# xiaochuanle/NECAT

Measured on AMD Instinct MI355X. Metric: overlaps/sec (all-vs-all, index build + seeding + banded Myers extension -> M4), higher is better.
Workload: dtype u64

## Files before the change

### necat_amd/csrc/knobs.h

```cpp
#pragma once
#include <stddef.h>
#include <stdint.h>
#include <stdlib.h>
#include <string>

#define NECAT_KNOBS(NUM, INT, SET, STR) \
     \
    NUM(index_lds,         int,    "NECAT_INDEX_LDS",         1, 0, ~0ull)            \
    NUM(split_threads,     ull,    "NECAT_SPLIT_THREADS",     512, 0, ~0ull)          \
    INT(index_own_offsets,         "NECAT_INDEX_OWN_OFFSETS", 0)                      \
    INT(index_emit_big,            "NECAT_INDEX_EMIT_BIG",    -1)                     \
    INT(index_dense_bases,         "NECAT_INDEX_DENSE_BASES", 0)                      \
    INT(no_lend,                   "NECAT_NO_LEND",          0)                      \
     \
    NUM(seed_budget,       ull,    "NECAT_SEED_BUDGET",       48ull << 20, 0, ~0ull)  \
    NUM(seed_wave,         int,    "NECAT_SEED_WAVE",         1, 0, ~0ull)            \
    NUM(seed_kst,          int,    "NECAT_SEED_KST",          1, 0, ~0ull)            \
    INT(seed_debug,                "NECAT_SEED_DEBUG",        0)                      \
    INT(chain_wave,                "NECAT_CHAIN_WAVE",        1)                      \
    SET(seed_clear_kernel,         "NECAT_SEED_CLEAR_KERNEL")                         \
     \
    NUM(batch_cap,         u32,    "NECAT_BATCH",             786432, 64, ~0ull)      \
     \
    NUM(ext_overlap,       u32,    "NECAT_EXT_OVERLAP",       1, 0, ~0ull) \
    NUM(ext_overlap_min,   u32,    "NECAT_EXT_OVERLAP_MIN",   0, 0, ~0ull) \
    NUM(ext_overlap_pct,   u32,    "NECAT_EXT_OVERLAP_PCT",   100, 0, 100) \
    NUM(ext_overlap_split, u32,    "NECAT_EXT_OVERLAP_SPLIT", 20, 5, 95) \
    NUM(ext_overlap_order, u32,    "NECAT_EXT_ORDER",         1, 0, ~0ull)            \
    NUM(ext_lanes,         u32,    "NECAT_EXT_LANES",         2, 1, kMaxExtLanes)     \
    INT(lane1_prio,                "NECAT_LANE1_PRIO",        1)                      \
    INT(serial,                    "NECAT_SERIAL",            0)                      \
    INT(stream_prio,               "NECAT_STREAM_PRIO",       0)                      \
     \
    NUM(coop_threshold,    u32,    "NECAT_COOP_THRESHOLD",    0xffffffffu, 0, ~0ull)  \
    NUM(coop_filter,       int,    "NECAT_COOP_FILTER",       1, 0, ~0ull)            \
    NUM(single_pass,       u32,    "NECAT_SINGLE_PASS",       4096, 0, ~0ull)         \
    NUM(sort_b,            int,    "NECAT_SORT_B",            1, 0, ~0ull)            \
    NUM(fast,              int,    "NECAT_FAST",              1, 0, ~0ull)            \
    NUM(fast16,            int,    "NECAT_FAST16",            0, 0, ~0ull)            \
    NUM(band_pool,         size_t, "NECAT_BAND_POOL_MB",      16384, 0, ~0ull)        \
    NUM(walk,              int,    "NECAT_WALK",              0, 0, ~0ull)            \
    NUM(walk_wave,         u32,    "NECAT_WALK_WAVE",         12288, 0, ~0ull)        \
    NUM(tail_fused,        u32,    "NECAT_TAIL_FUSED",        512, 0, ~0ull)          \
    NUM(dbg,               int,    "NECAT_DBG",               0, 0, ~0ull)            \
     \
    NUM(rcwalk,            u32,    "NECAT_RCWALK",            512, 0, ~0ull)          \
    NUM(rc_pool,           size_t, "NECAT_RC_POOL_MB",        8192, 1, ~0ull)         \
    NUM(rc_carry,          u32,    "NECAT_RC_CARRY",          1, 0, ~0ull)            \
    NUM(rc_listb,          u32,    "NECAT_RC_LISTB",          1, 0, ~0ull)            \
    NUM(rc_ragged,         u32,    "NECAT_RC_RAGGED",         1, 0, ~0ull)            \
    NUM(rc_merge,          u32,    "NECAT_RC_MERGE",          1, 0, ~0ull)            \
    NUM(frag_fuse,         u32,    "NECAT_FRAG_FUSE",         1, 0, ~0ull)            \
    NUM(item_sort,         u32,    "NECAT_ITEM_SORT",         1, 0, ~0ull)            \
    SET(rc_ckg_all,                "NECAT_RC_CKG_ALL")                                \
    NUM(rc_maxdist,        int,    "NECAT_RC_MAXDIST",        1 << 20, 0, ~0ull)      \
    NUM(ck_lds,            u32,    "NECAT_CK_LDS",            0, 0, ~0ull)            \
    NUM(ck_post,           u32,    "NECAT_CK_POST",           1, 0, ~0ull)            \
    NUM(ckr_fast,          u32,    "NECAT_CKR_FAST",          1, 0, ~0ull)            \
    NUM(rc_fastb,          u32,    "NECAT_RC_FASTB",          1, 0, ~0ull)            \
    NUM(rc_prio,           u32,    "NECAT_RC_PRIO",           1, 0, ~0ull)            \
     \
    NUM(rc_pipe,           u32,    "NECAT_RC_PIPE",           1, 1, 8) \
    NUM(rc_pipe_min,       u32,    "NECAT_RC_PIPE_MIN",       49152, 0, ~0ull) \
    NUM(rc_dbg,            u32,    "NECAT_RC_DBG",            0, 0, ~0ull)            \
    NUM(rc_prefetch,       u32,    "NECAT_RC_PREFETCH",       0, 0, ~0ull)            \
    NUM(rc_ww,             u32,    "NECAT_RC_WW",             1, 0, ~0ull)            \
    NUM(rc3_band,          ull,    "NECAT_RC3_BAND",          32, 0, ~0ull)           \
    NUM(rc3_min,           u32,    "NECAT_RC3_MIN",           160000, 0, ~0ull)       \
     \
    NUM(batch_chunk,       u32,    "NECAT_BATCH_CHUNK",       65536, 0, ~0ull)        \
    SET(batch_rc,                  "NECAT_BATCH_RC")                                  \
     \
    NUM(asm_rc,            u32,    "NECAT_ASM_RC",            1, 0, ~0ull)            \
    NUM(asm_rc_pool,       size_t, "NECAT_ASM_RC_POOL_MB",    2048, 256, ~0ull)       \
    NUM(asm_lane,          int,    "NECAT_ASM_LANE",          0, 0, ~0ull)            \
    NUM(asm_vote_budget,   ull,    "NECAT_ASM_VOTE_BUDGET",   16ull << 20, 1024, ~0ull)   \
    NUM(asm_seed_budget,   ull,    "NECAT_ASM_SEED_BUDGET",   32ull << 20, 1024, ~0ull)   \
    NUM(asm_ends_device,   int,    "NECAT_ASM_ENDS_DEVICE",   0, 0, 1)                \
    NUM(asm_ends_diags,    u32,    "NECAT_ASM_ENDS_DIAGS",    128, 4, 2048)           \
    SET(asm_no_overlap,            "NECAT_ASM_NO_OVERLAP")                            \
    STR(asm_dump_votes,            "NECAT_ASM_DUMP_VOTES")                            \
     \
    INT(cns_spec_extra,            "NECAT_CNS_SPEC_EXTRA",    1)                      \
    NUM(cns_spec_cover,    int,    "NECAT_CNS_SPEC",          12, 0, ~0ull)           \
    NUM(cns_device,        int,    "NECAT_CNS_DEVICE",        1, 0, 1)                \
    STR(cns_reads,                 "NECAT_CNS_READS")                                 \
    NUM(cns_chunk_bases,   ull,    "NECAT_CNS_CHUNK_BASES",   1ull << 31, 1, 1ull << 40)    \
    NUM(cns_tag_budget,    ull,    "NECAT_CNS_TAG_BUDGET",   32ull << 20, 1, 1ull << 30)   \
    NUM(cns_tol_scale,     ull,    "NECAT_CNS_TOL_SCALE",     1, 1, 1ull << 40)       \
    NUM(nw_device,         int,    "NECAT_NW_DEVICE",         0, 0, 1)                \
    NUM(nw_pool,           size_t, "NECAT_NW_POOL_MB",        1024, 1, 1ull << 20)    \
    NUM(dalign_device,     int,    "NECAT_DALIGN_DEVICE",     0, 0, 1)                \
    NUM(dalign_diags,      u32,    "NECAT_DALIGN_DIAGS",      512, 4, 2048)           \
    NUM(rm_rescue_device,  int,    "NECAT_RM_RESCUE_DEVICE",  0, 0, 1)                \
    NUM(ctg_seed_lds,      u32,    "NECAT_CTG_SEED_LDS",      512, 0, 2048)           \
    NUM(ctg_seed_budget,   ull,    "NECAT_CTG_SEED_BUDGET",   4ull << 20, 1, 1ull << 28)   \
    NUM(ctg_seed_job_max,  ull,    "NECAT_CTG_SEED_JOB_MAX",  16384, 1, 1ull << 28)        \
    INT(cns_threads,               "NECAT_CNS_THREADS",       32)                     \
    STR(comm,                      "NECAT_COMM")                                      \
    NUM(trace,             int,    "NECAT_TRACE",             0, 0, ~0ull)

namespace necat {

struct KnobSet { bool set; int v; };

struct Knobs {
    typedef uint32_t u32;
    typedef unsigned long long ull;
#define NECAT_KNOB_NUM(field, type, name, dflt, lo, hi) type field;
#define NECAT_KNOB_INT(field, name, dflt) int field;
#define NECAT_KNOB_SET(field, name) KnobSet field;
#define NECAT_KNOB_STR(field, name) std::string field;
    NECAT_KNOBS(NECAT_KNOB_NUM, NECAT_KNOB_INT, NECAT_KNOB_SET, NECAT_KNOB_STR)
};

extern thread_local const Knobs* tl_knobs;
inline const Knobs& knob() { return *tl_knobs; }

inline void index_plan_env(double* link_gbs, int* shard)
{
    const char *g = getenv("NECAT_XGMI_GBS"), *s = getenv("NECAT_INDEX_SHARD");
    *link_gbs = g && atof(g) > 0 ? atof(g) : 100.0; *shard = s ? atoi(s) != 0 : -1;
}

}
```

### necat_amd/csrc/necat_hip.hip

```cpp
#include <algorithm>
#include <chrono>
#include <memory>
#include <mutex>
#include <unordered_map>
#include <time.h>
#include <unistd.h>
#include <numeric>
#include <atomic>
#include <type_traits>

#ifdef NECAT_BUILD_CROSSCHECK
#define NECAT_XCHECK 1
#else
#define NECAT_XCHECK 0
#endif

#include "runtime.h"
#include "index_kernels.h"
#include "volume_kernels.h"
#include "seed_kernels.h"
#include "pcan_kernels.h"
#include "trim_kernels.h"
#include "ext_kernels.h"
#include "ext_tail.h"
#include "ext_rcwalk.h"
#include "ext_rcwalk3.h"
#include "asm_kernels.h"
#include "asm_coop.h"
#include "asm_plan.h"
#include "host_bases.h"
#include "host_threads.h"
#include "cns_loop.h"
#include "cns_rescue.h"
#include "cns_consensus.h"
#include "cns_dev_kernels.h"
#include "ctg_consensus.h"
#include "ctg_dev_kernels.h"
#include "ctg_seed.h"
#include "ctg_seed_kernels.h"
#include "ctg_extend.h"
#include "nw_kernels.h"
#include "dal_kernels.h"
#include "asm_ends_core.h"
#include "rm_host.h"
#include "rescue_pair.h"
#include "comm.h"
#include "pair_sched.h"


namespace necat { thread_local const Knobs* tl_knobs = nullptr; }
using namespace necat;

#define NECAT_RETIRED(ctx, what) return necat::set_err(ctx, NECAT_ERR_ARG, "%s: a cross-check path this library is built without (it is in libnecat_hip_xcheck.so, -DNECAT_BUILD_CROSSCHECK)", what)

static_assert(SC_COUNT <= (int)(sizeof(necat_ctx::scratch) / sizeof(necat::DevBuf)), "a ScratchId without an arena");

namespace {

int ensure_zeroed(necat_ctx* ctx, DevBuf& b, size_t bytes, hipStream_t s)
{
    const void* before = b.p; const size_t cap0 = b.cap;
    int rc = buf_ensure(ctx, b, bytes);
    if (rc) return rc;
    if (b.p != before || b.cap != cap0) { hipError_t e = hipMemsetAsync(b.p, 0, b.cap, s); if (e != hipSuccess) return set_err(ctx, NECAT_ERR_DEVICE, "memset failed"); }
    return NECAT_OK;
}

inline unsigned grid_for(uint64_t n, unsigned block, unsigned cap = 1u << 20)
{
    uint64_t g = (n + block - 1) / block;
    if (g < 1) g = 1;
    if (g > cap) g = cap;
    return (unsigned)g;
}

DevVolume dev_view(const necat_volume* v)
{
    DevVolume d; d.bases = v->bases; d.seq_off = v->seq_off; d.nbases = v->nbases; d.nseq = v->nseq;
    return d;
}


void finish_knobs(necat::Knobs& K)
{
    if (!K.rc_carry) { K.rc_listb = K.rc_ragged = 0; K.rc_maxdist = std::min(K.rc_maxdist, kRcMaxDist); }
    K.rc3_band = K.rc3_band == 16 ? 16 : 32;
    K.split_threads = K.split_threads == 256 ? 256 : 512;
    K.rc_dbg &= 6u;
    K.band_pool <<= 20; K.rc_pool <<= 20; K.asm_rc_pool <<= 20; K.nw_pool <<= 20;
    if (K.cns_threads <= 0) K.cns_threads = 32;
}

void read_knobs(necat::Knobs& K)
{
#define READ_NUM(field, type, name, dflt, lo, hi) { const char* e = getenv(name); K.field = (decltype(K.field))std::min<Knobs::ull>(hi, std::max<Knobs::ull>(lo, e ? strtoull(e, nullptr, 10) : (Knobs::ull)(dflt))); }
#define READ_INT(field, name, dflt) { const char* e = getenv(name); K.field = e ? atoi(e) : (dflt); }
#define READ_SET(field, name) { const char* e = getenv(name); K.field.set = e != nullptr; K.field.v = e ? atoi(e) : 0; }
#define READ_STR(field, name) { const char* e = getenv(name); K.field = e ? e : ""; }
    NECAT_KNOBS(READ_NUM, READ_INT, READ_SET, READ_STR)
    finish_knobs(K);
}

template <class T> int knob_text(char* buf, size_t n, T v) { if (std::is_signed<T>::value) snprintf(buf, n, "%lld", (long long)v); else snprintf(buf, n, "%llu", (unsigned long long)v); return NECAT_OK; }
int knob_text(char* buf, size_t n, const necat::KnobSet& v) { if (v.set) snprintf(buf, n, "%d", v.v); else buf[0] = 0; return NECAT_OK; }
int knob_text(char* buf, size_t n, const std::string& v) { snprintf(buf, n, "%s", v.c_str()); return NECAT_OK; }

double wall_ms() { struct timespec ts; clock_gettime(CLOCK_MONOTONIC, &ts); return ts.tv_sec * 1e3 + ts.tv_nsec * 1e-6; }

int fetch_words(necat_ctx* ctx, const necat_volume* v, std::vector<u64>* words)
{
    words->resize((v->nbases + 31) / 32 + 1);
    NECAT_HIP(ctx, hipMemcpy(words->data(), v->bases, (words->size() - 1) * 8, hipMemcpyDeviceToHost));
    return NECAT_OK;
}

int fetch_read_words(necat_ctx* ctx, const necat_volume* v, uint64_t id, std::vector<u64>* words, u64* word0)
{
    const u64 b = v->h_seq_off[id], e = v->h_seq_off[id + 1];
    *word0 = b >> 5;
    words->resize(e == b ? 0 : ((e - 1) >> 5) - *word0 + 1);
    if (!words->empty()) NECAT_HIP(ctx, hipMemcpy(words->data(), v->bases + *word0, words->size() * 8, hipMemcpyDeviceToHost));
    return NECAT_OK;
}

necat_host::BaseWords host_view(const necat_volume* v, const std::vector<u64>& words, u64 word0 = 0)
{
    necat_host::BaseWords b; b.w = words.data(); b.word0 = word0; b.seq_off = v->h_seq_off.data();
    return b;
}

unsigned call_threads(const necat_ctx* ctx, int host_threads)
{
    const unsigned want = host_threads ? (unsigned)std::min(host_threads, 256) : (unsigned)ctx->knobs.cns_threads;
    return std::max(1u, std::min(want, std::min(necat_host::hardware_threads(), 256u)));
}

struct SeqAt { int64_t k; u64 begin, len; };
bool seq_at(const necat_volume* v, int64_t id, int64_t start_id, SeqAt* s)
{
    s->k = id - start_id;
    if (s->k < 0 || (uint64_t)s->k >= v->nseq) return false;
    s->begin = v->h_seq_off[s->k]; s->len = v->h_seq_off[s->k + 1] - s->begin;
    return true;
}

int ctg_segment_check(necat_ctx* ctx, const necat_volume* contigs, const necat_ctg_segment& S, uint64_t s, int min_size, const char* what)
{
    if (S.size < 0 || S.from < 0 || S.ovlp_begin > S.ovlp_end) return set_err(ctx, NECAT_ERR_ARG, "segment %lu: bad size, start or %s range", (unsigned long)s, what);
    if ((int64_t)S.size >= necat_host::ctg::kMaxSegment) return set_err(ctx, NECAT_ERR_ARG, "segment %lu has %d bases: 2^24 or more", (unsigned long)s, S.size);
    if (S.size < min_size) return set_err(ctx, NECAT_ERR_ARG, "segment %lu has %d bases: fewer than %d, the reference has no defined answer", (unsigned long)s, S.size, min_size);
    SeqAt c;
    if (contigs && (!seq_at(contigs, S.ctg_id, 0, &c) || (u64)S.from + (u64)S.size > c.len)) return set_err(ctx, NECAT_ERR_ARG, "segment %lu leaves its contig", (unsigned long)s);
    return NECAT_OK;
}
static_assert(necat_host::ctg::kMaxSegment == necat_host::ctg_seed::kMaxSegment, "one bound on a segment for both contig stages");

}

#include "stage_ck_round.inl"

extern "C" {

void necat_default_options(necat_map_options* o)
{
    o->kmer_size = 15; o->scan_window = 10; o->kmer_cnt_cutoff = 500; o->block_size = 2000;
    o->block_score_cutoff = 3; o->num_candidates = 500; o->align_size_cutoff = 500;
    o->ddfs_cutoff = 0.25; o->error = 0.5; o->num_output = 500; o->num_threads = 1;
    o->job = 1; o->binary_output = 0; o->use_hdr_as_id = 1;
}

static thread_local char g_create_err[256] = "no context";
#define NECAT_CREATE_FAIL(code, ...) do { snprintf(g_create_err, sizeof g_create_err, __VA_ARGS__); return (code); } while (0)

int necat_ctx_create(int device_id, necat_ctx** out)
{
    if (!out) return NECAT_ERR_ARG;
    *out = nullptr;
    int ndev = 0;
    if (hipGetDeviceCount(&ndev) != hipSuccess || ndev <= 0) { (void)hipGetLastError(); NECAT_CREATE_FAIL(NECAT_ERR_DEVICE, "no usable HIP device (there is no CPU fallback)"); }
    if (device_id < 0 || device_id >= ndev) NECAT_CREATE_FAIL(NECAT_ERR_ARG, "device %d of %d", device_id, ndev);
    if (hipSetDevice(device_id) != hipSuccess) NECAT_CREATE_FAIL(NECAT_ERR_DEVICE, "hipSetDevice(%d) failed", device_id);
    necat_ctx* ctx = new necat_ctx();
    ctx->device = device_id;
    read_knobs(ctx->knobs);
#if !NECAT_XCHECK
    if (ctx->knobs.rc_ww == 0) {
        fprintf(stderr, "[necat] NECAT_RC_WW=0 selects k_rcwalk2, a cross-check kernel this library is built without (libnecat_hip_xcheck.so has it)\n");
        delete ctx; NECAT_CREATE_FAIL(NECAT_ERR_ARG, "NECAT_RC_WW=0 selects k_rcwalk2, a cross-check kernel this library is built without (libnecat_hip_xcheck.so has it)");
    }
#endif
    memset(&ctx->tm, 0, sizeof ctx->tm);
    memset(&ctx->shard_tm, 0, sizeof ctx->shard_tm);
    hipDeviceProp_t prop;
    if (hipGetDeviceProperties(&prop, device_id) == hipSuccess) {
        snprintf(ctx->devname, sizeof ctx->devname, "%s (%s), %d CUs", prop.name, prop.gcnArchName, prop.multiProcessorCount);
        ctx->num_cu = prop.multiProcessorCount;
    }
    if (hipStreamCreate(&ctx->stream) != hipSuccess) { delete ctx; return NECAT_ERR_DEVICE; }
    for (int i = 0; i < kNumEvents; ++i) if (hipEventCreate(&ctx->ev[i]) != hipSuccess) { delete ctx; return NECAT_ERR_DEVICE; }
    if (hipHostMalloc(&ctx->round_ring, kMaxExtLanes * kRoundRing * sizeof(RoundPub), hipHostMallocMapped | hipHostMallocCoherent) != hipSuccess ||
        hipHostGetDevicePointer(&ctx->round_ring_dev, ctx->round_ring, 0) != hipSuccess) { delete ctx; return NECAT_ERR_DEVICE; }
    memset(ctx->round_ring, 0, kMaxExtLanes * kRoundRing * sizeof(RoundPub));
    *out = ctx;
    return NECAT_OK;
}

void necat_ctx_destroy(necat_ctx* ctx)
{
    KnobScope knob_scope_(ctx);
    if (!ctx) return;
    (void)hipSetDevice(ctx->device);
    (void)hipStreamSynchronize(ctx->stream);
    if (knob().trace & 2) {
        size_t sum = 0; char own[1024]; int at = 0; own[0] = 0;
        for (int i = 0; i < (int)(sizeof ctx->scratch / sizeof ctx->scratch[0]); ++i) {
            sum += ctx->scratch[i].cap;
            if (ctx->scratch[i].cap >= ((size_t)64 << 20) && at < 980) at += snprintf(own + at, sizeof own - (size_t)at, " %d:%zu", i, ctx->scratch[i].cap >> 20);
        }
        fprintf(stderr, "[necat] context arenas at destroy: %zu MB in all; [id:MB]%s\n", sum >> 20, own);
    }
    if (ctx->stream_copy) (void)hipStreamSynchronize(ctx->stream_copy);
    for (auto& b : ctx->scratch) if (b.p) (void)hipFree(b.p);
    for (auto& b : ctx->idx_cache) if (b.p) (void)hipFree(b.p);
    if (ctx->cns_dev.p) (void)hipFree(ctx->cns_dev.p);
    for (auto& b : ctx->nw_buf) if (b.p) (void)hipFree(b.p);
    for (auto& b : ctx->dal_buf) if (b.p) (void)hipFree(b.p);
    for (auto& b : ctx->ctg_seed_buf) if (b.p) (void)hipFree(b.p);
    for (auto& lx : ctx->lanex) {
        for (auto& b : lx.buf) if (b.p) (void)hipFree(b.p);
        for (int i = 0; i < kNumEvents; ++i) if (lx.ev[i]) (void)hipEventDestroy(lx.ev[i]);
        for (hipStream_t st : lx.st) if (st) (void)hipStreamDestroy(st);
    }
    delete (cns::Scratch*)ctx->cns_scratch;
    if (ctx->pin_plan) (void)hipHostFree(ctx->pin_plan);
    for (int i = 0; i < kNumEvents; ++i) (void)hipEventDestroy(ctx->ev[i]);
    if (ctx->round_ring) (void)hipHostFree(ctx->round_ring);
    if (ctx->serial_streams) ctx->stream_a = ctx->stream_b = ctx->stream_c = ctx->stream_d = nullptr;
    for (hipStream_t st : {ctx->stream, ctx->stream_a, ctx->stream_b, ctx->stream_c, ctx->stream_d, ctx->stream_copy}) if (st) (void)hipStreamDestroy(st);
    delete ctx;
}

void necat_ctx_trim(necat_ctx* ctx)
{
    KnobScope knob_scope_(ctx);
    if (!ctx) return;
    (void)hipSetDevice(ctx->device);
    (void)hipDeviceSynchronize();
    for (auto& b : ctx->scratch) if (b.p) { (void)hipFree(b.p); b = DevBuf(); }
    for (auto& b : ctx->idx_cache) if (b.p) { (void)hipFree(b.p); b = DevBuf(); }
    if (ctx->cns_dev.p) { (void)hipFree(ctx->cns_dev.p); ctx->cns_dev = DevBuf(); }
    for (auto& b : ctx->nw_buf) if (b.p) { (void)hipFree(b.p); b = DevBuf(); }
    for (auto& b : ctx->dal_buf) if (b.p) { (void)hipFree(b.p); b = DevBuf(); }
    for (auto& b : ctx->ctg_seed_buf) if (b.p) { (void)hipFree(b.p); b = DevBuf(); }
    for (auto& lx : ctx->lanex) for (auto& b : lx.buf) if (b.p) { (void)hipFree(b.p); b = DevBuf(); }
    ctx->seed_ht_ptr = nullptr; ctx->seed_ht_clean = 0; ctx->seed_ht_cap = 0;
}

const char* necat_last_error(const necat_ctx* ctx) { return ctx ? ctx->err : g_create_err; }

int necat_device_name(const necat_ctx* ctx, char* buf, size_t n)
{
    KnobScope knob_scope_(ctx);
    if (!ctx || !buf || !n) return NECAT_ERR_ARG;
    snprintf(buf, n, "%s", ctx->devname);
    return NECAT_OK;
}

int necat_get_timings(const necat_ctx* ctx, necat_timings* t)
{
    KnobScope knob_scope_(ctx);
    if (!ctx || !t) return NECAT_ERR_ARG;
    *t = ctx->tm;
    return NECAT_OK;
}

int necat_get_timings_sized(const necat_ctx* ctx, void* t, size_t bytes)
{
    KnobScope knob_scope_(ctx);
    if (!ctx || !t) return NECAT_ERR_ARG;
    memcpy(t, &ctx->tm, bytes < sizeof(necat_timings) ? bytes : sizeof(necat_timings));
    return NECAT_OK;
}

int necat_get_rm_stats_sized(const necat_ctx* ctx, void* stats, size_t bytes)
{
    KnobScope knob_scope_(ctx);
    if (!ctx || !stats) return NECAT_ERR_ARG;
    memcpy(stats, &ctx->rm_stats, bytes < sizeof(necat_rm_stats) ? bytes : sizeof(necat_rm_stats));
    return NECAT_OK;
}

int necat_get_item_order_stats(const necat_ctx* ctx, necat_item_order_stats* stats)
{
    if (!ctx || !stats) return NECAT_ERR_ARG;
    *stats = ctx->item_order;
    return NECAT_OK;
}

int necat_knob_get(const necat_ctx* ctx, const char* name, char* buf, size_t n)
{
    KnobScope knob_scope_(ctx);
    if (!ctx || !name || !buf || !n) return NECAT_ERR_ARG;
#define GET_KNOB(field, env) if (!strcmp(name, env)) return knob_text(buf, n, ctx->knobs.field);
#define GET_NUM(field, type, env, dflt, lo, hi) GET_KNOB(field, env)
#define GET_INT(field, env, dflt) GET_KNOB(field, env)
    NECAT_KNOBS(GET_NUM, GET_INT, GET_KNOB, GET_KNOB)
    return NECAT_ERR_ARG;
}

int necat_abi_version(void) { return NECAT_ABI_VERSION; }

namespace {
struct ResultPool {
    std::mutex mu;
    std::unordered_map<void*, size_t> live;
    std::vector<std::pair<void*, size_t>> parked;
};
ResultPool g_results;
constexpr size_t kPinnedMin = 256 << 10, kPoolBlocks = 16, kPoolBytes = (size_t)8 << 30;

void* result_alloc(size_t bytes)
{
    if (bytes < kPinnedMin) return malloc(bytes ? bytes : 1);
    std::lock_guard<std::mutex> lk(g_results.mu);
    int best = -1;
    for (int i = 0; i < (int)g_results.parked.size(); ++i) {
        const size_t sz = g_results.parked[i].second;
        if (sz >= bytes && sz <= 2 * bytes + (1 << 20) && (best < 0 || sz < g_results.parked[best].second)) best = i;
    }
    void* p = nullptr; size_t sz = 0;
    if (best >= 0) { p = g_results.parked[best].first; sz = g_results.parked[best].second; g_results.parked.erase(g_results.parked.begin() + best); }
    else {
        sz = (bytes + (bytes >> 3) + 4095) & ~(size_t)4095;
        if (hipHostMalloc(&p, sz, hipHostMallocDefault) != hipSuccess) { (void)hipGetLastError(); return malloc(bytes); }
    }
    g_results.live[p] = sz;
    return p;
}
}

void necat_free(void* p)
{
    if (!p) return;
    {
        std::lock_guard<std::mutex> lk(g_results.mu);
        auto it = g_results.live.find(p);
        if (it != g_results.live.end()) {
            const size_t sz = it->second;
            g_results.live.erase(it);
            g_results.parked.emplace_back(p, sz);
            size_t held = 0;
            for (auto& b : g_results.parked) held += b.second;
            while (g_results.parked.size() > kPoolBlocks || (held > kPoolBytes && !g_results.parked.empty())) {
                size_t k = 0;
                for (size_t i = 1; i < g_results.parked.size(); ++i) if (g_results.parked[i].second < g_results.parked[k].second) k = i;
                held -= g_results.parked[k].second;
                (void)hipHostFree(g_results.parked[k].first);
                g_results.parked.erase(g_results.parked.begin() + k);
            }
            return;
        }
    }
    free(p);
}

#include "stage_volumes.inl"
#include "stage_index.inl"
#include "stage_seed.inl"
#include "stage_extend.inl"
#include "stage_asm_align.inl"
#include "stage_asm_plan.inl"
#include "stage_pcan.inl"
#include "stage_trim.inl"
#include "stage_multi.inl"
#include "stage_align_batch.inl"
#include "stage_nw.inl"
#include "stage_dalign.inl"
#include "stage_refmap.inl"
#include "stage_asm_ends.inl"
#include "stage_cns.inl"
#include "stage_cns_consensus.inl"
#include "stage_ctg_consensus.inl"
#include "stage_ctg_seed.inl"
#include "stage_ctg_extend.inl"
#include "stage_edlib_batch.inl"

}
```

### necat_amd/csrc/runtime.h

```cpp
#pragma once
#include <hip/hip_runtime.h>
#include <assert.h>
#include <stdarg.h>
#include <stdio.h>
#include <stdlib.h>
#include <string.h>

#include <initializer_list>
#include <string>
#include <utility>
#include <vector>

#include "../../include/necat_hip.h"
#include "knobs.h"
#include "dev_common.h"
#include "stage_arenas.h"

namespace necat {

struct DevBuf {
    void* p = nullptr;
    size_t cap = 0;
};

}

constexpr int kNumEvents = 48;
enum EventId {
    EV_CALL_BEGIN = 0, EV_CALL_END = 1,
    EV_ASM_A0 = 2, EV_ASM_A1 = 3,
    EV_A0 = 4, EV_A1 = 5, EV_A2 = 6,
    EV_EDLIB_A0 = EV_A0, EV_EDLIB_A1 = EV_A1, EV_EDLIB_A2 = EV_A2,
    EV_COLS_READY = 16, EV_COLS_COPIED = 17,
    EV_B0 = 18, EV_B1 = 19, EV_B2 = 20,
    EV_ASM_A2 = 24,
    EV_SIDE_CHAIN = 25,
    EV_RC_WALK_END = 26,
    EV_RAGGED_WALKED = 30,
    EV_LANE_RESULT = 31,
    EV_ASM_FORK = 34, EV_ASM_JOIN = 35,
    EV_ASM_B0 = 36, EV_ASM_B1 = 37, EV_ASM_B2 = 38,
    EV_PIPE_PIECE = 40,
};
constexpr int kEvListStride = 3, kEvRcRounds = 4, kEvPipePieces = 8;
struct EvRange { int first, count; };
constexpr EvRange kEvRanges[] = {{EV_CALL_BEGIN, 2}, {EV_ASM_A0, 2}, {EV_A0, kEvListStride * 4}, {EV_COLS_READY, 2}, {EV_B0, kEvListStride * 2}, {EV_ASM_A2, 1}, {EV_SIDE_CHAIN, 1},
                                 {EV_RC_WALK_END, kEvRcRounds}, {EV_RAGGED_WALKED, 1}, {EV_LANE_RESULT, 1}, {EV_ASM_FORK, 2}, {EV_ASM_B0, 3}, {EV_PIPE_PIECE, kEvPipePieces}};
constexpr bool ev_ranges_disjoint() { int end = 0; for (const EvRange& r : kEvRanges) { if (r.first < end) return false; end = r.first + r.count; } return end <= kNumEvents; }
static_assert(ev_ranges_disjoint(), "two owners of one event index, or a range past kNumEvents (kEvRanges is in ascending order)");
static_assert(EV_CALL_END == EV_CALL_BEGIN + 1 && EV_ASM_A1 == EV_ASM_A0 + 1 && EV_A2 == EV_A0 + 2 && EV_B2 == EV_B0 + 2 && EV_COLS_COPIED == EV_COLS_READY + 1 &&
              EV_ASM_JOIN == EV_ASM_FORK + 1 && EV_ASM_B2 == EV_ASM_B0 + 2 && EV_EDLIB_A0 == EV_A0 && EV_EDLIB_A2 == EV_A2, "the ranges above are these names' ranges");
constexpr unsigned kRoundRing = 1024;
constexpr int kMaxExtLanes = 4;

struct ExtLane1 {
    necat::DevBuf buf[16];
    hipStream_t st[4] = {nullptr, nullptr, nullptr, nullptr};
    hipEvent_t ev[kNumEvents] = {};
    unsigned long long round_seq = 0;
    bool ready = false;
};

struct necat_ctx {
    int device = 0;
    hipStream_t stream = nullptr;
    hipStream_t stream_a = nullptr, stream_b = nullptr;
    hipStream_t stream_c = nullptr;
    hipStream_t stream_d = nullptr;
    bool serial_streams = false;
    hipStream_t stream_copy = nullptr;
    bool copy_pending = false;
    char err[1024] = {0};
    necat_timings tm;
    necat_shard_timings shard_tm;
    hipEvent_t ev[kNumEvents];
    void* pin_plan = nullptr; size_t pin_plan_cap = 0;
    void* round_ring = nullptr;
    void* round_ring_dev = nullptr;
    unsigned long long round_seq = 0;
    necat::DevBuf scratch[64];
    uint64_t scratch_live = 0;
    void* seed_ht_ptr = nullptr;
    size_t seed_ht_cap = 0;
    size_t seed_ht_clean = 0;
    char devname[256] = {0};
    int num_cu = 0;
    uint32_t epoch = 0;
    void* cns_scratch = nullptr;
    necat::Knobs knobs;
    necat::DevBuf idx_cache[4];
    ExtLane1 lanex[kMaxExtLanes - 1];
    int trim_nids = 0;
    uint64_t trim_total = 0;
    necat::DevBuf nw_buf[8];
    necat::DevBuf dal_buf[5];
    double dal_error = 0.0; int dal_ave_path = 0;
    double gather_ms = 0; uint64_t gather_bytes = 0;
    necat_item_order_stats item_order = {};
    necat_rm_stats rm_stats = {};
    necat::DevBuf cns_dev;
    necat::DevBuf ctg_seed_buf[3];
};

constexpr int kIdxCacheHoles = 2;

struct necat_volume {
    uint64_t nbases = 0, nseq = 0;
    uint64_t* bases_alloc = nullptr;
    uint64_t* bases = nullptr;
    uint64_t* seq_off = nullptr;
    std::vector<uint64_t> h_seq_off;
};

struct necat_index {
    int k = 0;
    uint64_t table_entries = 0, n_offsets = 0;
    void* table = nullptr;
    uint64_t* kmer_stats = nullptr;
    void* words = nullptr;
    uint64_t* compact = nullptr;
    uint64_t n_compact = 0;
    uint64_t* offset_list = nullptr;
    size_t stats_cap = 0, offs_cap = 0;
    uint64_t n_slices = 0, offsets_cap = 0, compact_cap = 0;
    uint64_t* slice_start = nullptr;
    uint32_t *slice_kept = nullptr, *slice_pres = nullptr;
};

namespace necat {

struct KnobScope {
    const Knobs* prev;
    explicit KnobScope(const necat_ctx* c) : prev(tl_knobs) { if (c) tl_knobs = &c->knobs; }
    ~KnobScope() { tl_knobs = prev; }
    KnobScope(const KnobScope&) = delete; KnobScope& operator=(const KnobScope&) = delete;
};

inline int set_err(necat_ctx* ctx, int code, const char* fmt, ...)
{
    if (ctx) {
        va_list ap; va_start(ap, fmt);
        vsnprintf(ctx->err, sizeof ctx->err, fmt, ap);
        va_end(ap);
    }
    return code;
}

#define NECAT_HIP(ctx, call) do { hipError_t e__ = (call); if (e__ != hipSuccess) \
    return necat::set_err(ctx, NECAT_ERR_DEVICE, "%s failed: %s (%s:%d)", #call, hipGetErrorString(e__), __FILE__, __LINE__); } while (0)

#define NECAT_CHECK_LAUNCH(ctx, name) do { hipError_t e__ = hipGetLastError(); if (e__ != hipSuccess) \
    return necat::set_err(ctx, NECAT_ERR_DEVICE, "launch of %s failed: %s", name, hipGetErrorString(e__)); } while (0)

constexpr int kGuardWords = 4;

inline int buf_ensure(necat_ctx* ctx, DevBuf& b, size_t bytes)
{
    if (bytes <= b.cap) return NECAT_OK;
    if (b.p) { hipError_t e = hipFree(b.p); (void)e; b.p = nullptr; b.cap = 0; }
    size_t want = bytes + bytes / 8 + 256;
    hipError_t e = hipMalloc(&b.p, want);
    if (e != hipSuccess) {
        b.p = nullptr; b.cap = 0;
        size_t fr = 0, tot = 0;
        if (hipMemGetInfo(&fr, &tot) != hipSuccess) fr = tot = 0;
        char own[512]; int at = 0; size_t sum = 0;
        own[0] = 0;
        if (ctx) for (int i = 0; i < (int)(sizeof ctx->scratch / sizeof ctx->scratch[0]); ++i) {
            sum += ctx->scratch[i].cap;
            if (ctx->scratch[i].cap >= ((size_t)256 << 20) && at < 480) at += snprintf(own + at, sizeof own - (size_t)at, " %d:%zu", i, ctx->scratch[i].cap >> 20);
        }
        return set_err(ctx, NECAT_ERR_MEMORY, "hipMalloc(%zu) failed: %s (device memory: %zu MB free of %zu MB; this context's arenas: %zu MB, the big ones [id:MB]%s)", want,
                       hipGetErrorString(e), fr >> 20, tot >> 20, sum >> 20, own);
    }
    b.cap = want;
    return NECAT_OK;
}

inline int buf_grow(necat_ctx* ctx, DevBuf& b, size_t bytes, size_t keep, hipStream_t s)
{
    if (bytes <= b.cap) return NECAT_OK;
    size_t want = bytes > 2 * b.cap ? bytes + bytes / 8 + 256 : 2 * b.cap;
    void* q = nullptr;
    hipError_t e = hipMalloc(&q, want);
    if (e != hipSuccess) return set_err(ctx, NECAT_ERR_MEMORY, "hipMalloc(%zu) failed: %s", want, hipGetErrorString(e));
    if (b.p && keep) {
        e = hipMemcpyAsync(q, b.p, keep, hipMemcpyDeviceToDevice, s);
        if (e == hipSuccess) e = hipStreamSynchronize(s);
        if (e != hipSuccess) { (void)hipFree(q); return set_err(ctx, NECAT_ERR_DEVICE, "device copy failed: %s", hipGetErrorString(e)); }
    }
    if (b.p) (void)hipFree(b.p);
    b.p = q; b.cap = want;
    return NECAT_OK;
}

template <class T> inline T* as(const DevBuf& b) { return (T*)b.p; }

struct ArenaView {
    char* base; size_t total; hipStream_t s;
    ArenaView(const DevBuf& b, const ArenaLayout& l, hipStream_t st) : base((char*)b.p), total(l.bytes()), s(st) { assert(total <= b.cap); }
    template <class T> T* ptr(Span<T> sp) const { assert(sp.end() <= total); return (T*)(base + sp.off); }
    template <class T> const T* cptr(Span<T> sp) const { return ptr(sp); }
    template <class T> hipError_t upload(Span<T> sp, const T* src, size_t n) const { assert(n <= sp.n); return hipMemcpyAsync(ptr(sp), src, n * sizeof(T), hipMemcpyHostToDevice, s); }
    template <class T> hipError_t download(T* dst, Span<T> sp, size_t n, size_t first = 0) const { assert(first + n <= sp.n); return hipMemcpyAsync(dst, ptr(sp) + first, n * sizeof(T), hipMemcpyDeviceToHost, s); }
    template <class T> hipError_t fill(Span<T> sp, int byte, size_t n) const { assert(n <= sp.n); return hipMemsetAsync(ptr(sp), byte, n * sizeof(T), s); }
    template <class T> hipError_t zero(Span<T> sp, size_t n) const { return fill(sp, 0, n); }
    template <class T> hipError_t zero_from(Span<T> sp) const { assert(sp.off <= total); return hipMemsetAsync(base + sp.off, 0, total - sp.off, s); }
};

inline double ev_ms(hipEvent_t a, hipEvent_t b) { float ms = 0; if (hipEventElapsedTime(&ms, a, b) != hipSuccess) return 0; return ms; }

template <int N>
struct CallEvents {
    hipEvent_t ev[N] = {};
    CallEvents() = default;
    CallEvents(const CallEvents&) = delete; CallEvents& operator=(const CallEvents&) = delete;
    ~CallEvents() { for (auto& e : ev) if (e) (void)hipEventDestroy(e); }
    int create(necat_ctx* ctx) { for (auto& e : ev) NECAT_HIP(ctx, hipEventCreate(&e)); return NECAT_OK; }
    hipError_t record(int i, hipStream_t s) const { return hipEventRecord(ev[i], s); }
    double ms(int i) const { return ev_ms(ev[i], ev[i + 1]); }
};

struct ResultOwner {
    void* held[2] = {nullptr, nullptr}; int n = 0;
    ResultOwner() = default;
    ResultOwner(const ResultOwner&) = delete; ResultOwner& operator=(const ResultOwner&) = delete;
    ~ResultOwner() { for (int i = 0; i < n; ++i) necat_free(held[i]); }
    template <class T> T* own(void* p) { assert(n < 2); held[n++] = p; return (T*)p; }
    void release() { n = 0; }
};

enum ScratchId {
    SC_CNT32 = 0, SC_PARTIAL, SC_TMPLIST, SC_MISC,
    SC_SEED_META, SC_SEED_HT, SC_SEED_POOL, SC_SEED_CHAIN, SC_SEED_OUT, SC_SEED_FINAL,
    SC_EXT_TASKS, SC_EXT_LISTS, SC_EXT_FRAG, SC_EXT_MAT, SC_EXT_OPS, SC_EXT_RES, SC_EXT_CAND, SC_SMALL, SC_PART,
    SC_EXT_COLS, SC_EXT_COLS_OUT, SC_PART2, SC_SEED_ALL, SC_EXT_MATB, SC_EXT_MATB2, SC_EXT_PERM, SC_GATHER, SC_SPLIT, SC_SPLIT2,
    SC_ASM_BAND, SC_ASM_OPS, SC_ASM_COLS, SC_ASM_MISC, SC_ASM_FRAG, SC_ASM_OUT, SC_SEED_KST, SC_EXT_CKPT, SC_EXT_WOUT, SC_EXT_CKPTB, SC_EXT_CKPTB2, SC_EXT_WOUTB, SC_EXT_WOUTB2,
    SC_ASM_OCC, SC_ASM_TAB, SC_ASM_VMETA, SC_ASM_VHT, SC_ASM_VPOOL, SC_ASM_VOUT, SC_ASM_SEL, SC_ASM_RIDX, SC_ASM_RNEXT, SC_ASM_PAIRS, SC_ASM_SEEDS,
    SC_ASM_VMETA2, SC_ASM_VHT2, SC_ASM_VPOOL2, SC_ASM_VOUT2, SC_ASM_SEL2, SC_ASM_RIDX2, SC_ASM_RNEXT2,
    SC_STATS,
    SC_TRIM_IN, SC_TRIM_RECS, SC_TRIM_OFF,
    SC_COUNT
};

struct ArenaUse {
    necat_ctx* ctx; uint64_t mine;
    ArenaUse(necat_ctx* c, std::initializer_list<int> ids) : ctx(c), mine(0) { for (int i : ids) mine |= 1ULL << i; mine &= ~c->scratch_live; c->scratch_live |= mine; }
    ~ArenaUse() { ctx->scratch_live &= ~mine; }
    ArenaUse(const ArenaUse&) = delete; ArenaUse& operator=(const ArenaUse&) = delete;
};
inline int buf_ensure_lend(necat_ctx* ctx, int id, size_t bytes, std::initializer_list<int> donors)
{
    DevBuf& b = ctx->scratch[id];
    if (bytes <= b.cap) return NECAT_OK;
    if (!ctx->knobs.no_lend) for (int d : donors) {
        DevBuf& o = ctx->scratch[d];
        if (d != id && o.cap >= bytes && !((ctx->scratch_live >> d) & 1ULL)) { std::swap(b, o); return NECAT_OK; }
    }
    return buf_ensure(ctx, b, bytes);
}

}
```

Measured before the change: 6.829 million.

## Create list-A/list-B streams with priorities at context creation

Context creation now builds a set of streams up front: a primary stream shared with list A, one or two streams for list B, and optionally a stream for the ragged/piped chain, with configurable priority classes. List B defaults to the lowest priority. Teardown is changed to destroy each distinct stream exactly once, since streams may now alias. The intent is to let list A and list B work overlap with explicit scheduling priority rather than creating streams lazily. The risk is that low priority on list B delays its completion, or that the extra streams add contention.

```diff
diff --git a/necat_amd/csrc/knobs.h b/necat_amd/csrc/knobs.h
--- a/necat_amd/csrc/knobs.h
+++ b/necat_amd/csrc/knobs.h
@@ -31,6 +31,10 @@
     INT(lane1_prio,                "NECAT_LANE1_PRIO",        1)                      \
     INT(serial,                    "NECAT_SERIAL",            0)                      \
     INT(stream_prio,               "NECAT_STREAM_PRIO",       0)                      \
+     \
+    NUM(stream_graph,      u32,    "NECAT_STREAM_GRAPH",      1, 0, 1) \
+    INT(listb_prio,                "NECAT_LISTB_PRIO",        1) \
+    NUM(listb_streams,     u32,    "NECAT_LISTB_STREAMS",     2, 1, 2) \
      \
     NUM(coop_threshold,    u32,    "NECAT_COOP_THRESHOLD",    0xffffffffu, 0, ~0ull)  \
     NUM(coop_filter,       int,    "NECAT_COOP_FILTER",       1, 0, ~0ull)            \
diff --git a/necat_amd/csrc/necat_hip.hip b/necat_amd/csrc/necat_hip.hip
--- a/necat_amd/csrc/necat_hip.hip
+++ b/necat_amd/csrc/necat_hip.hip
@@ -107,6 +107,39 @@
 
 double wall_ms() { struct timespec ts; clock_gettime(CLOCK_MONOTONIC, &ts); return ts.tv_sec * 1e3 + ts.tv_nsec * 1e-6; }
 
+hipError_t make_stream(hipStream_t* st, int cls)
+{
+    int least = 0, greatest = 0;
+    if (cls && hipDeviceGetStreamPriorityRange(&least, &greatest) != hipSuccess) { (void)hipGetLastError(); least = greatest = 0; }
+    return cls && least != greatest ? hipStreamCreateWithPriority(st, hipStreamDefault, cls == 1 ? least : greatest) : hipStreamCreate(st);
+}
+
+int ctx_streams(necat_ctx* ctx)
+{
+    const necat::Knobs& K = ctx->knobs;
+    ctx->need_stream_d = NECAT_XCHECK || !(K.rc_merge && K.rc_ragged && K.rc_carry && !K.rc_ckg_all.set) || K.rc_pipe > 1;
+    ctx->graph_streams = K.stream_graph && !K.serial;
+    if (!ctx->graph_streams) return hipStreamCreate(&ctx->stream) == hipSuccess ? NECAT_OK : NECAT_ERR_DEVICE;
+    const int cls_a = K.stream_prio == 2 ? 2 : 0;
+    const int cls_b = K.stream_prio == 1 ? 2 : K.listb_prio == 1 || K.listb_prio == 2 ? K.listb_prio : 0;
+    if (make_stream(&ctx->stream, cls_a) != hipSuccess) return NECAT_ERR_DEVICE;
+    ctx->stream_a = ctx->stream;
+    if (make_stream(&ctx->stream_b, cls_b) != hipSuccess) return NECAT_ERR_DEVICE;
+    if (K.listb_streams < 2) ctx->stream_c = ctx->stream_b;
+    else if (make_stream(&ctx->stream_c, cls_b) != hipSuccess) return NECAT_ERR_DEVICE;
+    if (ctx->need_stream_d && make_stream(&ctx->stream_d, cls_b) != hipSuccess) return NECAT_ERR_DEVICE;
+    if (K.trace)
+        fprintf(stderr, "[necat] context streams (NECAT_STREAM_GRAPH=1): %d made - its own and list A's (priority class %d), %d for list B (class %d)%s; classes: 0 normal, 1 lowest, 2 highest\n",
+                1 + (K.listb_streams < 2 ? 1 : 2) + (ctx->need_stream_d ? 1 : 0), cls_a, K.listb_streams < 2 ? 1 : 2, cls_b, ctx->need_stream_d ? ", 1 for the ragged / piped chain (list B's class)" : "");
+    return NECAT_OK;
+}
+
+void destroy_streams(std::initializer_list<hipStream_t> all)
+{
+    std::vector<hipStream_t> seen;
+    for (hipStream_t st : all) if (st && std::find(seen.begin(), seen.end(), st) == seen.end()) { seen.push_back(st); (void)hipStreamDestroy(st); }
+}
+
 int fetch_words(necat_ctx* ctx, const necat_volume* v, std::vector<u64>* words)
 {
     words->resize((v->nbases + 31) / 32 + 1);
@@ -196,7 +229,10 @@
         snprintf(ctx->devname, sizeof ctx->devname, "%s (%s), %d CUs", prop.name, prop.gcnArchName, prop.multiProcessorCount);
         ctx->num_cu = prop.multiProcessorCount;
     }
-    if (hipStreamCreate(&ctx->stream) != hipSuccess) { delete ctx; return NECAT_ERR_DEVICE; }
+    if (ctx_streams(ctx) != NECAT_OK) {
+        destroy_streams({ctx->stream, ctx->stream_a, ctx->stream_b, ctx->stream_c, ctx->stream_d});
+        delete ctx; NECAT_CREATE_FAIL(NECAT_ERR_DEVICE, "hipStreamCreate failed");
+    }
     for (int i = 0; i < kNumEvents; ++i) if (hipEventCreate(&ctx->ev[i]) != hipSuccess) { delete ctx; return NECAT_ERR_DEVICE; }
     if (hipHostMalloc(&ctx->round_ring, kMaxExtLanes * kRoundRing * sizeof(RoundPub), hipHostMallocMapped | hipHostMallocCoherent) != hipSuccess ||
         hipHostGetDevicePointer(&ctx->round_ring_dev, ctx->round_ring, 0) != hipSuccess) { delete ctx; return NECAT_ERR_DEVICE; }
@@ -229,14 +265,13 @@
     for (auto& lx : ctx->lanex) {
         for (auto& b : lx.buf) if (b.p) (void)hipFree(b.p);
         for (int i = 0; i < kNumEvents; ++i) if (lx.ev[i]) (void)hipEventDestroy(lx.ev[i]);
-        for (hipStream_t st : lx.st) if (st) (void)hipStreamDestroy(st);
+        destroy_streams({lx.st[0], lx.st[1], lx.st[2], lx.st[3]});
     }
     delete (cns::Scratch*)ctx->cns_scratch;
     if (ctx->pin_plan) (void)hipHostFree(ctx->pin_plan);
     for (int i = 0; i < kNumEvents; ++i) (void)hipEventDestroy(ctx->ev[i]);
     if (ctx->round_ring) (void)hipHostFree(ctx->round_ring);
-    if (ctx->serial_streams) ctx->stream_a = ctx->stream_b = ctx->stream_c = ctx->stream_d = nullptr;
-    for (hipStream_t st : {ctx->stream, ctx->stream_a, ctx->stream_b, ctx->stream_c, ctx->stream_d, ctx->stream_copy}) if (st) (void)hipStreamDestroy(st);
+    destroy_streams({ctx->stream, ctx->stream_a, ctx->stream_b, ctx->stream_c, ctx->stream_d, ctx->stream_copy});
     delete ctx;
 }
 
diff --git a/necat_amd/csrc/runtime.h b/necat_amd/csrc/runtime.h
--- a/necat_amd/csrc/runtime.h
+++ b/necat_amd/csrc/runtime.h
@@ -68,6 +68,8 @@
     hipStream_t stream_c = nullptr;
     hipStream_t stream_d = nullptr;
     bool serial_streams = false;
+    bool graph_streams = false;
+    bool need_stream_d = true;
     hipStream_t stream_copy = nullptr;
     bool copy_pending = false;
     char err[1024] = {0};
```

Result: faster. 8.185 million (median of 6 runs) (+19.9%).
